# E3SM-Project/Omega

Hardware: AMD Instinct MI355X
Metric: tendency_cell_level_updates_per_sec (higher is better)
Workload: dtype f64

## Files before the change

### include/omega_amd.h

```cpp
#ifndef OMEGA_AMD_H
#define OMEGA_AMD_H

#include <stddef.h>
#include <stdint.h>

#ifdef __cplusplus
extern "C" {
#endif

typedef struct omg_decomp omg_decomp;
typedef struct omg_halo omg_halo;
typedef struct omg_mesh omg_mesh;
typedef struct omg_state omg_state;
typedef struct omg_tracers omg_tracers;
typedef struct omg_aux omg_aux;
typedef struct omg_tend omg_tend;
typedef struct omg_stepper omg_stepper;
typedef struct omg_vcoord omg_vcoord;
typedef struct omg_eos omg_eos;
typedef struct omg_vertmix omg_vertmix;
typedef struct omg_pgrad omg_pgrad;
typedef struct omg_vertadv omg_vertadv;

enum { OMG_ON_CELL = 0, OMG_ON_EDGE = 1, OMG_ON_VERTEX = 2 };
// ... 88 lines not shown
typedef struct omg_rccl omg_rccl;
int omg_rccl_get_unique_id(char *id );
int omg_rccl_create(const char *id, int nranks, int rank, omg_rccl **out);
int omg_rccl_destroy(omg_rccl *c);
int omg_rccl_abort(omg_rccl *c);
int omg_rccl_info(const omg_rccl *c, int *nranks, int *rank, int *version, int64_t *exchanges);
int omg_rccl_exchange(omg_rccl *c, int n, const int *peers, void *const *send_ptrs, const size_t *send_bytes,
                      void *const *recv_ptrs, const size_t *recv_bytes, void *stream);
int omg_halo_use_rccl(omg_halo *h, omg_rccl *c);
enum { OMG_PEER_HANDLE_BYTES = 160 };
typedef struct omg_peer omg_peer;
int omg_peer_create(int nranks, int rank, size_t mailbox_bytes, omg_peer **out);
int omg_peer_destroy(omg_peer *p);
int omg_peer_local_handle(const omg_peer *p, char *out );
int omg_peer_connect(omg_peer *p, const char *all_handles );
int omg_peer_info(const omg_peer *p, int64_t *exchanges, int *status);
int omg_peer_set_timeout(omg_peer *p, double seconds);
int omg_halo_use_peer(omg_halo *h, omg_peer *p);
int omg_halo_recv_rows(const omg_halo *h, size_t per_cell, size_t per_edge, size_t per_vertex, size_t *rows);
int omg_halo_exchange(omg_halo *h, double *dev_array, int nt, int rows_size, int k, int row_pitch, int elem,
                      void *stream);
int omg_halo_exchange_bytes(omg_halo *h, void *dev_array, int elem_bytes, int nt, int rows_size, int k, int row_pitch,
                            int elem, void *stream);
int omg_halo_exchange_i4(omg_halo *h, int32_t *dev_array, int nt, int rows_size, int k, int row_pitch, int elem,
                         void *stream);
int omg_halo_global_sum_dd(omg_halo *h, const double *local_hi_lo, int npairs, double *hi_lo, void *stream);
int omg_halo_exchange_state(omg_halo *h, omg_state *state, int state_time_level, omg_tracers *tracers,
                            int tracers_time_level, void *stream);
int omg_halo_check(const omg_halo *h);

int omg_set_option(const char *name, int value);
int omg_get_option(const char *name, int *value);
int omg_set_timing_level(int level);

int omg_mesh_create(const omg_decomp *d, int nvertlayers, int host_only, omg_mesh **out);
int omg_mesh_destroy(omg_mesh *m);
int omg_mesh_get_int(const omg_mesh *m, const char *name, int32_t *out);
int omg_mesh_get_array_i4(const omg_mesh *m, const char *name, int32_t *out, size_t n);
int omg_mesh_get_array_r8(const omg_mesh *m, const char *name, double *out, size_t n);
int omg_mesh_set_fvertex(omg_mesh *m, const double *host_values );

int omg_horz_divergence(const omg_mesh *m, const double *vec_edge_dev, double *div_cell_dev, int nvertlayers,
                        int row_pitch, int n, void *stream);
int omg_horz_gradient(const omg_mesh *m, const double *scalar_cell_dev, double *grad_edge_dev, int nvertlayers,
                      int row_pitch, int n, void *stream);
int omg_horz_curl(const omg_mesh *m, const double *vec_edge_dev, double *curl_vertex_dev, int nvertlayers,
                  int row_pitch, int n, void *stream);
int omg_horz_tangential_recon(const omg_mesh *m, const double *vec_edge_dev, double *recon_edge_dev, int nvertlayers,
                              int row_pitch, int n, void *stream);
int omg_horz_interp_cell_to_edge(const omg_mesh *m, const double *array_cell_dev, double *array_edge_dev,
                                 int isotropic, int n, void *stream);

typedef struct omg_tend_config {
   int32_t ThicknessFluxTendencyEnable, PVTendencyEnable, KETendencyEnable, SSHTendencyEnable,
       VelDiffTendencyEnable, VelHyperDiffTendencyEnable, WindForcingTendencyEnable, BottomDragTendencyEnable,
       TracerHorzAdvTendencyEnable, TracerDiffTendencyEnable, TracerHyperDiffTendencyEnable;
   int32_t FluxThicknessUpwind, FluxTracerUpwind, WindInterpIsotropic;
   double ViscDel2, ViscDel4, DivFactor, EddyDiff2, EddyDiff4, Density0, BottomDragCoeff;
} omg_tend_config;
void omg_tend_config_default(omg_tend_config *c);

int omg_state_create(const omg_mesh *m, omg_halo *halo, int nvertlayers, int ntimelevels, omg_state **out);
int omg_state_destroy(omg_state *s);
int omg_state_copy_to_device(omg_state *s, int time_level, const double *h_host, const double *u_host);
int omg_state_copy_to_host(const omg_state *s, int time_level, double *h_host, double *u_host);
int omg_state_device_ptr(const omg_state *s, int time_level, int which , double **dev);
// ... 172 lines not shown
```

### omega_amd/__init__.py

```python
from __future__ import annotations

import ctypes as C
import os
import subprocess

import numpy as np

_HERE = os.path.dirname(os.path.abspath(__file__))
LIB_PATH = os.environ.get("OMEGA_AMD_LIB", os.path.join(_HERE, "lib", "libomega_amd.so"))

ON_CELL, ON_EDGE, ON_VERTEX = 0, 1, 2

PD = C.POINTER(C.c_double)
PI = C.POINTER(C.c_int32)


class OmegaAmdError(RuntimeError):
    pass


def build(force: bool = False) -> str:
    cmd = ["make", "-C", os.path.join(_HERE, "csrc"), "-j8", "-s"]
    if force:
        cmd.append("-B")
# ... 20 lines not shown


class TendConfig(C.Structure):
    _fields_ = [(n, C.c_int32) for n in CONFIG_FLAGS] + [(n, C.c_double) for n in CONFIG_REALS]


TRANSPORT_FN = C.CFUNCTYPE(C.c_int, C.c_void_p, C.c_int, PI, C.POINTER(C.c_void_p), C.POINTER(C.c_size_t),
                           C.POINTER(C.c_void_p), C.POINTER(C.c_size_t), C.c_void_p)

CUSTOM_TEND_FN = C.CFUNCTYPE(C.c_int, C.c_void_p, C.c_void_p, C.c_void_p, C.c_void_p, C.c_int, C.c_int, C.c_int,
                             C.c_int, C.c_double, C.c_void_p)

_lib = None


def lib():
    global _lib
    if _lib is None:
        if not os.path.exists(LIB_PATH):
            raise OmegaAmdError(
                f"{LIB_PATH} not found: build it with `python -c 'import __graft_entry__ as g; g.build()'` "
                "(hipcc, gfx950). omega_amd has no CPU fallback.")
        L = C.CDLL(LIB_PATH)
        L.omg_last_error.restype = C.c_char_p
        _lib = L
        for item in filter(None, os.environ.get("OMEGA_AMD_OPTIONS", "").split(",")):
            name, _, val = item.partition("=")
            set_option(name.strip(), int(val))
    return _lib


def set_option(name: str, value: int):
    _chk(lib().omg_set_option(name.encode(), int(value)))


def get_option(name: str) -> int:
    v = C.c_int()
    _chk(lib().omg_get_option(name.encode(), C.byref(v)))
    return v.value


def _chk(rc):
    if rc != 0:
        raise OmegaAmdError(lib().omg_last_error().decode())


def _pd(a):
    if a is None:
        return PD()
    assert a.dtype == np.float64 and a.flags.c_contiguous, "need C-contiguous float64"
    return a.ctypes.data_as(PD)


def _pi(a):
    if a is None:
        return PI()
    assert a.dtype == np.int32 and a.flags.c_contiguous, "need C-contiguous int32"
    return a.ctypes.data_as(PI)


class _Handle:
    _destroy = None

    def _create(self, symbol: str, *args):
        h = C.c_void_p()
        _chk(getattr(lib(), symbol)(*args, C.byref(h)))
# ... 1171 lines not shown
```

### omega_amd/csrc/Device.cpp

```cpp
#include "Base.h"
#include "Pacer.h"
#include "Tuning.h"

#include <rocprofiler-sdk-roctx/roctx.h>

#include <atomic>
#include <cctype>
#include <cstdlib>

#include <cstring>
#include <sstream>

namespace OMEGA {

namespace {
struct OptionName {
   const char *Name;
   int TuningOptions::*Field;
};
const OptionName OptionTable[] = {
    {"MergeL1", &TuningOptions::MergeL1},
    {"Pair", &TuningOptions::Pair},
    {"TracerPatch", &TuningOptions::TracerPatch},
    {"SendBand", &TuningOptions::SendBand},
// ... 12 lines not shown
#ifdef OMEGA_TUNING_ENV
      for (const OptionName &O : OptionTable) {
         std::string Var = "OMEGA_";
         for (const char *C = O.Name; *C; ++C)
            Var += (char)std::toupper((unsigned char)*C);
         if (const char *V = std::getenv(Var.c_str()))
            X.*(O.Field) = std::atoi(V);
      }
#endif
      return X;
   }();
   return T;
}
namespace {
std::atomic<unsigned long long> TuningGen{0};
}
unsigned long long tuningGeneration() { return TuningGen.load(); }
bool setTuningOption(const std::string &Name, int Value) {
   for (const OptionName &O : OptionTable)
      if (Name == O.Name) {
         tuning().*(O.Field) = Value;
         ++TuningGen;
         return true;
      }
   return false;
}
bool getTuningOption(const std::string &Name, int &Value) {
   for (const OptionName &O : OptionTable)
      if (Name == O.Name) {
         Value = tuning().*(O.Field);
         return true;
      }
   return false;
}

namespace Pacer {
int &timingLevel() {
   static int Level = 3;
   return Level;
}
namespace {
constexpr int MaxLevels = 16;
thread_local int PushedAt[MaxLevels] = {};
int slot(int Level) { return Level < 0 ? 0 : (Level >= MaxLevels ? MaxLevels - 1 : Level); }
}
bool start(const char *Name, int Level) {
   if (Level <= timingLevel()) {
      roctxRangePushA(Name);
      if (Level > -1000000)
         ++PushedAt[slot(Level)];
   }
   return true;
}
bool stop(const char * , int Level) {
   if (Level <= -1000000) {
      roctxRangePop();
      return true;
   }
   if (PushedAt[slot(Level)] > 0) {
      --PushedAt[slot(Level)];
      roctxRangePop();
   }
   return true;
}
}

// ... 85 lines not shown
```

### omega_amd/csrc/Tuning.h

```cpp
#ifndef OMEGA_AMD_TUNING_H
#define OMEGA_AMD_TUNING_H

#include <string>

namespace OMEGA {

struct TuningOptions {
   int MergeL1 = 1;
   int Pair = 1;
   int TracerPatch = 1;
   int SendBand = 1;
   int BandOnComm = 1;
   int ShrinkSweeps = 1;
   int ForceGeneric = 0;
   int KeepMaxEdges = 0;
   int NarrowTables = 1;
   int Graphs = -1;
};

TuningOptions &tuning();
unsigned long long tuningGeneration();
bool setTuningOption(const std::string &Name, int Value);
bool getTuningOption(const std::string &Name, int &Value);

}
#endif
```

### omega_amd/csrc/capi.cpp

```cpp
#include "../../include/omega_amd.h"

#include "AuxiliaryState.h"
#include "Decomp.h"
#include "Halo.h"
#include "HorzMesh.h"
#include "HorzOperators.h"
#include "OceanState.h"
#include "Tendencies.h"
#include "CustomTendencyTerms.h"
#include "MeshIO.h"
#include "Partition.h"
#include "History.h"
#include "Pacer.h"
#include "PeerWire.h"
#include "Rccl.h"
#include "Tuning.h"
#include "TimeStepper.h"
#include "VertCoord.h"
#include "Eos.h"
#include "TriDiagSolvers.h"
#include "VertMix.h"
#include "PressureGrad.h"
#include "VertAdv.h"

// ... 544 lines not shown
   if (version)
      *version = c->C->Version;
   if (exchanges)
      *exchanges = c->C->NExchanges;
   OMG_CATCH
}
int omg_rccl_exchange(omg_rccl *c, int n, const int *peers, void *const *send_ptrs, const size_t *send_bytes,
                      void *const *recv_ptrs, const size_t *recv_bytes, void *stream) {
   OMG_TRY
   OMG_ARG(c && n >= 0 && (n == 0 || (peers && send_ptrs && send_bytes && recv_ptrs && recv_bytes)));
   if (c->C->exchange(n, peers, send_ptrs, send_bytes, recv_ptrs, recv_bytes, (hipStream_t)stream) != 0)
      OMEGA_ABORT(c->C->lastError());
   OMG_CATCH
}
int omg_halo_use_rccl(omg_halo *h, omg_rccl *c) {
   OMG_TRY
   OMG_ARG(h && c);
   h->H->useRccl(c->C.get());
   OMG_CATCH
}
int omg_set_option(const char *name, int value) {
   OMG_TRY
   OMG_ARG(name);
   if (!setTuningOption(name, value))
      OMEGA_ABORT(std::string("omg_set_option: no option named '") + name + "'");
   OMG_CATCH
}
int omg_get_option(const char *name, int *value) {
   OMG_TRY
   OMG_ARG(name && value);
   if (!getTuningOption(name, *value))
      OMEGA_ABORT(std::string("omg_get_option: no option named '") + name + "'");
   OMG_CATCH
}
int omg_set_timing_level(int level) {
   Pacer::timingLevel() = level;
   return 0;
}
int omg_peer_create(int nranks, int rank, size_t mailbox_bytes, omg_peer **out) {
   OMG_TRY
   OMG_ARG(out);
   newHandle(out, [&](omg_peer &R) { R.P.reset(new PeerWire(nranks, rank, mailbox_bytes)); });
   OMG_CATCH
}
int omg_peer_destroy(omg_peer *p) {
   delete p;
   return 0;
}
int omg_peer_local_handle(const omg_peer *p, char *out) {
   OMG_TRY
   OMG_ARG(p && out);
   p->P->localHandle(out);
   OMG_CATCH
}
int omg_peer_connect(omg_peer *p, const char *all_handles) {
   OMG_TRY
   OMG_ARG(p && all_handles);
   p->P->connect(all_handles);
   OMG_CATCH
}
int omg_peer_info(const omg_peer *p, int64_t *exchanges, int *status) {
   OMG_TRY
   OMG_ARG(p);
   if (exchanges)
      *exchanges = p->P->NExchanges;
   if (status)
// ... 1126 lines not shown
```

### omega_amd/csrc/kernels/KernelCommon.h

```cpp
#ifndef OMEGA_AMD_KERNELCOMMON_H
#define OMEGA_AMD_KERNELCOMMON_H

#include <cstdlib>
#include <type_traits>
#include <utility>
#include <hip/hip_runtime.h>

#include "../Base.h"
#include "../Tuning.h"

namespace OMEGA {

typedef double dv2 __attribute__((ext_vector_type(2)));

template <class T> struct VecW;
template <> struct VecW<double> {
   static constexpr int W = 1;
};
template <> struct VecW<dv2> {
   static constexpr int W = 2;
};

template <class T> __device__ __forceinline__ T ldk(const double *P, int Row, int K, int Kv) {
   return *reinterpret_cast<const T *>(P + (size_t)Row * K + (size_t)Kv * VecW<T>::W);
}
template <class T> __device__ __forceinline__ void stk(double *P, int Row, int K, int Kv, T V) {
   *reinterpret_cast<T *>(P + (size_t)Row * K + (size_t)Kv * VecW<T>::W) = V;
}

__device__ __forceinline__ double kmax(double A, double B) { return A < B ? B : A; }
__device__ __forceinline__ dv2 kmax(dv2 A, dv2 B) {
   dv2 R;
   R.x = kmax(A.x, B.x);
   R.y = kmax(A.y, B.y);
   return R;
}
__device__ __forceinline__ double upwind(double U, double A, double B) {
   return U > 0 ? A : (U < 0 ? B : kmax(A, B));
}
__device__ __forceinline__ dv2 upwind(dv2 U, dv2 A, dv2 B) {
   dv2 R;
   R.x = upwind(U.x, A.x, B.x);
   R.y = upwind(U.y, A.y, B.y);
   return R;
}
template <class T> __device__ __forceinline__ T splat(double V);
template <> __device__ __forceinline__ double splat<double>(double V) { return V; }
template <> __device__ __forceinline__ dv2 splat<dv2>(double V) {
   dv2 R;
   R.x = V;
   R.y = V;
   return R;
}

__device__ __forceinline__ double getc(double V, int) { return V; }
__device__ __forceinline__ double getc(dv2 V, int I) { return I == 0 ? V.x : V.y; }
__device__ __forceinline__ void setc(double &V, int, double X) { V = X; }
__device__ __forceinline__ void setc(dv2 &V, int I, double X) {
   if (I == 0)
      V.x = X;
   else
      V.y = X;
}

__device__ __forceinline__ int xcdRemap(int B, int N) {
   const int Q = N >> 3, R = N & 7;
   const int Xcd = B & 7, Idx = B >> 3;
   return (Xcd < R ? Xcd * (Q + 1) : R * (Q + 1) + (Xcd - R) * Q) + Idx;
}

struct LdsCarver {
   unsigned char *P;
   template <class U> __device__ __forceinline__ U *take(int N) {
      U *R = reinterpret_cast<U *>(P);
      P += (((size_t)N * sizeof(U) + 7) >> 3) << 3;
      return R;
   }
};
__host__ __device__ inline size_t ldsRound8(size_t B) { return ((B + 7) >> 3) << 3; }

struct Geom {
   dim3 Grid, Block;
   int KV;
   int Tile;
   int W;
   int NFull = 0, TailSplit = 1;
};
inline Geom makeGeom(int N, int K, int MaxW = 2, int Pitch = 0, int MaxTY = 0) {
   if (Pitch <= 0)
      Pitch = K;
   Geom G;
   G.W  = (K % 2 == 0 && MaxW >= 2) ? 2 : 1;
   G.KV = K / G.W;
   const int LineTX   = 128 / (8 * G.W);
   const bool Aligned = (Pitch * 8) % 128 == 0;
   int TX             = Aligned ? (G.KV < LineTX ? G.KV : LineTX) : (G.KV < 64 ? G.KV : 64);
   int TY = 256 / TX;
   while (MaxTY > 0 && TY > MaxTY && TY > 8)
      TY /= 2;
   while (TY > 8 && (N + TY - 1) / TY < 4096)
      TY /= 2;
   if (TY < 1)
      TY = 1;
   G.Block = dim3(TX, TY, 1);
   G.Tile  = TY;
   int NTiles = (N + G.Tile - 1) / G.Tile;
   int NChunks = (G.KV + TX - 1) / TX, Split = 1;
   while (Split < NChunks && (long)NTiles * Split < 1200)
      Split *= 2;
   if (Split > NChunks)
      Split = NChunks;
   G.Grid  = dim3(NTiles > 0 ? NTiles : 1, Split > 0 ? Split : 1, 1);
   G.NFull = NTiles;
   const int WavesPerWG     = (TX * TY + 63) / 64;
   const int Cap            = 256 * 8 / (WavesPerWG > 0 ? WavesPerWG : 1);
   if (Split == 1 && NChunks > 1 && NTiles >= Cap) {
      const int R = NTiles % Cap;
      if (R > 0) {
         G.NFull     = NTiles - R;
         G.TailSplit = NChunks;
         G.Grid      = dim3(G.NFull + R * NChunks, 1, 1);
      }
   }
   return G;
}

template <class B, class = void> struct BodyHoistTables {
   static constexpr bool V = false;
};
template <class B> struct BodyHoistTables<B, std::enable_if_t<B::HoistTables>> {
   static constexpr bool V = true;
};
template <class B> __device__ __forceinline__ void chunkFence() {
#ifndef OMEGA_NO_CHUNK_FENCE
   if constexpr (!BodyHoistTables<B>::V)
      __asm__ volatile("" ::: "memory");
#endif
}
template <class B, class = void> struct BodyOpaqueLe {
   static constexpr bool V = false;
};
template <class B> struct BodyOpaqueLe<B, std::enable_if_t<B::OpaqueLe>> {
   static constexpr bool V = true;
};
template <class B, class = void> struct BodyCooperative {
   static constexpr bool V = false;
};
template <class B> struct BodyCooperative<B, std::enable_if_t<B::Cooperative>> {
   static constexpr bool V = true;
};
template <class B, class = void> struct BodyMinWaves {
   static constexpr int V = 1;
};
template <class B> struct BodyMinWaves<B, decltype((void)B::MinWaves)> {
   static constexpr int V = B::MinWaves;
};
template <class B, class = void> struct BodyMaxW {
   static constexpr int V = 2;
// ... 20 lines not shown
   }
   const int First = TileId * Tile;
   int Cnt          = N - First;
   if (Cnt > Tile)
      Cnt = Tile;
   typename Body::Lds L = B.carve(Lds, Tile);
   const int Tid        = threadIdx.y * blockDim.x + threadIdx.x;
   const int NThr       = blockDim.x * blockDim.y;
   if (Cnt > 0)
      B.stage(L, First, Cnt, Tid, NThr);
   __syncthreads();
#ifdef OMEGA_STAGE_ONLY
   return;
#endif
   if constexpr (BodyCooperative<Body>::V) {
      B.template computeTile<T>(L, First, Cnt, C0, CS, KV);
   } else {
      for (int Le = threadIdx.y; Le < Cnt; Le += blockDim.y)
         for (int Kv = C0 * blockDim.x + threadIdx.x; Kv < KV; Kv += blockDim.x * CS) {
            chunkFence<Body>();
            if constexpr (BodyOpaqueLe<Body>::V) {
               int LeO = Le;
               __asm__ volatile("" : "+v"(LeO));
               B.template compute<T>(L, LeO, First + Le, Kv);
            } else
               B.template compute<T>(L, Le, First + Le, Kv);
         }
   }
}

template <class BA, class BB, class T>
__global__ void __launch_bounds__(OMEGA_LB, (BodyMinWaves<BA>::V < BodyMinWaves<BB>::V ? BodyMinWaves<BA>::V
                                                                                       : BodyMinWaves<BB>::V))
    tileKernel2(BA A, BB Bb, int NA, int NB, int KV, int Tile, int NTilesA, int NFullB, int TailSplit) {
   extern __shared__ __align__(16) unsigned char Lds[];
   const int Tid  = threadIdx.y * blockDim.x + threadIdx.x;
   const int NThr = blockDim.x * blockDim.y;
   if ((int)blockIdx.x < NTilesA) {
      const int Ta    = xcdRemap(blockIdx.x, NTilesA);
      const int First = Ta * Tile;
      const int Cnt   = NA - First < Tile ? NA - First : Tile;
      typename BA::Lds L = A.carve(Lds, Tile);
      if (Cnt > 0)
         A.stage(L, First, Cnt, Tid, NThr);
      __syncthreads();
#ifdef OMEGA_STAGE_ONLY
      return;
#endif
      for (int Le = threadIdx.y; Le < Cnt; Le += blockDim.y)
         for (int Kv = blockIdx.y * blockDim.x + threadIdx.x; Kv < KV; Kv += blockDim.x * gridDim.y)
         {
            chunkFence<BA>();
            A.template compute<T>(L, Le, First + Le, Kv);
         }
   } else {
      const int Bb_ = blockIdx.x - NTilesA;
      int TileId, C0 = blockIdx.y, CS = gridDim.y;
      if (Bb_ < NFullB) {
         TileId = xcdRemap(Bb_, NFullB);
      } else {
         TileId = NFullB + (Bb_ - NFullB) / TailSplit;
         C0     = (Bb_ - NFullB) % TailSplit;
         CS     = TailSplit;
      }
      const int First = TileId * Tile;
      const int Cnt   = NB - First < Tile ? NB - First : Tile;
      typename BB::Lds L = Bb.carve(Lds, Tile);
      if (Cnt > 0)
         Bb.stage(L, First, Cnt, Tid, NThr);
      __syncthreads();
#ifdef OMEGA_STAGE_ONLY
      return;
#endif
      for (int Le = threadIdx.y; Le < Cnt; Le += blockDim.y)
         for (int Kv = C0 * blockDim.x + threadIdx.x; Kv < KV; Kv += blockDim.x * CS)
         {
            chunkFence<BB>();
            Bb.template compute<T>(L, Le, First + Le, Kv);
         }
   }
}

template <class B, class = void> struct BodyHasNT {
   static constexpr bool V = false;
};
template <class B> struct BodyHasNT<B, decltype((void)std::declval<B &>().NT)> {
   static constexpr bool V = true;
};
template <class B> inline int bodyMaxTY(const B &Body) {
   if constexpr (BodyHasNT<B>::V)
      return Body.NT <= 8 ? 16 : 0;
   else
      return 0;
}
template <class B, class = void> struct BodyHasKLog {
   static constexpr bool V = false;
};
template <class B> struct BodyHasKLog<B, decltype((void)std::declval<B &>().KLog)> {
   static constexpr bool V = true;
};
template <class B, class = void> struct BodyHasNWv {
   static constexpr bool V = false;
};
template <class B> struct BodyHasNWv<B, decltype((void)std::declval<B &>().NWv)> {
   static constexpr bool V = true;
};
template <class B> inline void setWaves(B &Body, const Geom &G) {
   if constexpr (BodyHasNWv<B>::V)
      Body.NWv = (int)(G.Block.x * G.Block.y + 63) / 64;
}
template <class Body> void launchTile(const Body &B0, int N, int K, hipStream_t S, int Pitch = -1) {
   if (N <= 0)
      return;
   Body B = B0;
   B.K    = Pitch > 0 ? Pitch : levelPitch(K);
   if constexpr (BodyHasKLog<Body>::V)
      B.KLog = K;
   Geom G           = makeGeom(N, K, BodyMaxW<Body>::V, B.K, bodyMaxTY(B));
   setWaves(B, G);
   const size_t Lds = B.ldsBytes(G.Tile);
   if constexpr (BodyMaxW<Body>::V >= 2) {
      if (G.W == 2) {
         hipLaunchKernelGGL((tileKernel<Body, dv2>), G.Grid, G.Block, Lds, S, B, N, G.KV, G.Tile, G.NFull, G.TailSplit);
         HIP_CHECK(hipGetLastError());
         return;
      }
   }
   hipLaunchKernelGGL((tileKernel<Body, double>), G.Grid, G.Block, Lds, S, B, N, G.KV, G.Tile, G.NFull, G.TailSplit);
   HIP_CHECK(hipGetLastError());
}

template <class BA, class BB> void launchTile2(const BA &A0, int NA, const BB &B0, int NB, int K, hipStream_t S) {
   static_assert(BodyMaxW<BA>::V == BodyMaxW<BB>::V, "launchTile2: bodies must agree on the levels per thread");
   if (NA <= 0) {
      launchTile(B0, NB, K, S);
      return;
   }
   if (NB <= 0) {
      launchTile(A0, NA, K, S);
      return;
   }
   BA A  = A0;
   BB Bb = B0;
   A.K = Bb.K = levelPitch(K);
   if constexpr (BodyHasKLog<BA>::V)
      A.KLog = K;
   if constexpr (BodyHasKLog<BB>::V)
      Bb.KLog = K;
   const int TyA = bodyMaxTY(A), TyB = bodyMaxTY(Bb);
   Geom G        = makeGeom(NA + NB, K, BodyMaxW<BA>::V, A.K, TyA > TyB ? TyA : TyB);
   const int NTA = (NA + G.Tile - 1) / G.Tile, NTB = (NB + G.Tile - 1) / G.Tile;
   setWaves(A, G), setWaves(Bb, G);
   const size_t LA = A.ldsBytes(G.Tile), LB = Bb.ldsBytes(G.Tile), Lds = LA > LB ? LA : LB;
   int NFullB = NTB, TailSplit = 1;
   dim3 Grid(NTA + NTB, G.TailSplit > 1 ? 1 : G.Grid.y, 1);
   if (G.TailSplit > 1) {
      const int R = (NTA + NTB) - G.NFull;
      if (R > 0 && R <= NTB) {
         NFullB    = NTB - R;
         TailSplit = G.TailSplit;
         Grid      = dim3(NTA + NFullB + R * TailSplit, 1, 1);
      }
   }
   if constexpr (BodyMaxW<BA>::V >= 2) {
      if (G.W == 2) {
         hipLaunchKernelGGL((tileKernel2<BA, BB, dv2>), Grid, G.Block, Lds, S, A, Bb, NA, NB, G.KV, G.Tile, NTA, NFullB,
                            TailSplit);
         HIP_CHECK(hipGetLastError());
         return;
      }
   }
   hipLaunchKernelGGL((tileKernel2<BA, BB, double>), Grid, G.Block, Lds, S, A, Bb, NA, NB, G.KV, G.Tile, NTA, NFullB,
                      TailSplit);
   HIP_CHECK(hipGetLastError());
}

constexpr int MaxSweeps = 4;
struct SweepPlan {
   int N[MaxSweeps];
   int TileStart[MaxSweeps + 1];
};
template <int I, class T, class B, class... Rest>
__device__ __forceinline__ void runSweep(const SweepPlan &Pl, int KV, int Tile, unsigned char *Lds, const B &Body,
                                         const Rest &...More) {
   if ((int)blockIdx.x < Pl.TileStart[I + 1]) {
      const int NTiles = Pl.TileStart[I + 1] - Pl.TileStart[I];
      const int Tl     = xcdRemap(blockIdx.x - Pl.TileStart[I], NTiles);
      const int First  = Tl * Tile;
      const int Cnt    = Pl.N[I] - First < Tile ? Pl.N[I] - First : Tile;
      typename B::Lds L = Body.carve(Lds, Tile);
      const int Tid     = threadIdx.y * blockDim.x + threadIdx.x;
      if (Cnt > 0)
         Body.stage(L, First, Cnt, Tid, blockDim.x * blockDim.y);
      __syncthreads();
      if constexpr (BodyCooperative<B>::V) {
         Body.template computeTile<T>(L, First, Cnt, blockIdx.y, gridDim.y, KV);
      } else {
         for (int Le = threadIdx.y; Le < Cnt; Le += blockDim.y)
            for (int Kv = blockIdx.y * blockDim.x + threadIdx.x; Kv < KV; Kv += blockDim.x * gridDim.y) {
               chunkFence<B>();
               Body.template compute<T>(L, Le, First + Le, Kv);
            }
      }
      return;
   }
   if constexpr (sizeof...(Rest) > 0)
      runSweep<I + 1, T>(Pl, KV, Tile, Lds, More...);
}
template <class... Bs> struct MinWavesOf;
template <class B> struct MinWavesOf<B> {
   static constexpr int V = BodyMinWaves<B>::V;
};
template <class B, class... Bs> struct MinWavesOf<B, Bs...> {
   static constexpr int V = BodyMinWaves<B>::V < MinWavesOf<Bs...>::V ? BodyMinWaves<B>::V : MinWavesOf<Bs...>::V;
};
template <class T, class... Bs>
__global__ void __launch_bounds__(OMEGA_LB, MinWavesOf<Bs...>::V) tileKernelV(SweepPlan Pl, int KV, int Tile, Bs... Bodies) {
   extern __shared__ __align__(16) unsigned char Lds[];
   runSweep<0, T>(Pl, KV, Tile, Lds, Bodies...);
}

namespace detail {
template <class B> inline void prepBody(B &Body, int K) {
   Body.K = levelPitch(K);
   if constexpr (BodyHasKLog<B>::V)
      Body.KLog = K;
}
}
template <class B0, class B1> void launchTileV(int K, hipStream_t S, const B0 &A0, int N0, const B1 &A1, int N1) {
   static_assert(BodyMaxW<B0>::V == BodyMaxW<B1>::V, "launchTileV: bodies must agree on the levels per thread");
   static_assert(sizeof(B0) + sizeof(B1) + sizeof(SweepPlan) <= 3900, "launchTileV: kernel arguments exceed 4 KiB");
   B0 X0 = A0;
   B1 X1 = A1;
   detail::prepBody(X0, K), detail::prepBody(X1, K);
   const int Ns[2] = {N0 > 0 ? N0 : 0, N1 > 0 ? N1 : 0};
   const int Ty0 = bodyMaxTY(X0), Ty1 = bodyMaxTY(X1);
   Geom G = makeGeom(Ns[0] + Ns[1], K, BodyMaxW<B0>::V, X0.K, Ty0 > Ty1 ? Ty0 : Ty1);
   SweepPlan Pl{};
   Pl.TileStart[0] = 0;
   for (int I = 0; I < 2; ++I) {
      Pl.N[I]             = Ns[I];
      Pl.TileStart[I + 1] = Pl.TileStart[I] + (Ns[I] + G.Tile - 1) / G.Tile;
   }
   if (Pl.TileStart[2] == 0)
      return;
   setWaves(X0, G), setWaves(X1, G);
   const size_t L0 = X0.ldsBytes(G.Tile), L1 = X1.ldsBytes(G.Tile), Lds = L0 > L1 ? L0 : L1;
   const dim3 Grid(Pl.TileStart[2], G.TailSplit > 1 ? 1 : G.Grid.y, 1);
   if constexpr (BodyMaxW<B0>::V >= 2) {
      if (G.W == 2) {
         hipLaunchKernelGGL((tileKernelV<dv2, B0, B1>), Grid, G.Block, Lds, S, Pl, G.KV, G.Tile, X0, X1);
         HIP_CHECK(hipGetLastError());
         return;
      }
   }
   hipLaunchKernelGGL((tileKernelV<double, B0, B1>), Grid, G.Block, Lds, S, Pl, G.KV, G.Tile, X0, X1);
   HIP_CHECK(hipGetLastError());
}
template <class B0, class B1, class B2>
void launchTileV(int K, hipStream_t S, const B0 &A0, int N0, const B1 &A1, int N1, const B2 &A2, int N2) {
   static_assert(BodyMaxW<B0>::V == BodyMaxW<B1>::V && BodyMaxW<B0>::V == BodyMaxW<B2>::V,
                 "launchTileV: bodies must agree on the levels per thread");
   static_assert(sizeof(B0) + sizeof(B1) + sizeof(B2) + sizeof(SweepPlan) <= 3900, "launchTileV: kernel arguments exceed 4 KiB");
   B0 X0 = A0;
   B1 X1 = A1;
   B2 X2 = A2;
   detail::prepBody(X0, K), detail::prepBody(X1, K), detail::prepBody(X2, K);
   const int Ns[3] = {N0 > 0 ? N0 : 0, N1 > 0 ? N1 : 0, N2 > 0 ? N2 : 0};
   int Ty = bodyMaxTY(X0);
   Ty     = bodyMaxTY(X1) > Ty ? bodyMaxTY(X1) : Ty;
   Ty     = bodyMaxTY(X2) > Ty ? bodyMaxTY(X2) : Ty;
   Geom G = makeGeom(Ns[0] + Ns[1] + Ns[2], K, BodyMaxW<B0>::V, X0.K, Ty);
   SweepPlan Pl{};
   Pl.TileStart[0] = 0;
   for (int I = 0; I < 3; ++I) {
      Pl.N[I]             = Ns[I];
      Pl.TileStart[I + 1] = Pl.TileStart[I] + (Ns[I] + G.Tile - 1) / G.Tile;
   }
   if (Pl.TileStart[3] == 0)
      return;
   setWaves(X0, G), setWaves(X1, G), setWaves(X2, G);
   size_t Lds = X0.ldsBytes(G.Tile);
   Lds        = X1.ldsBytes(G.Tile) > Lds ? X1.ldsBytes(G.Tile) : Lds;
   Lds        = X2.ldsBytes(G.Tile) > Lds ? X2.ldsBytes(G.Tile) : Lds;
   const dim3 Grid(Pl.TileStart[3], G.TailSplit > 1 ? 1 : G.Grid.y, 1);
   if constexpr (BodyMaxW<B0>::V >= 2) {
      if (G.W == 2) {
         hipLaunchKernelGGL((tileKernelV<dv2, B0, B1, B2>), Grid, G.Block, Lds, S, Pl, G.KV, G.Tile, X0, X1, X2);
         HIP_CHECK(hipGetLastError());
         return;
      }
   }
   hipLaunchKernelGGL((tileKernelV<double, B0, B1, B2>), Grid, G.Block, Lds, S, Pl, G.KV, G.Tile, X0, X1, X2);
   HIP_CHECK(hipGetLastError());
}

}
#endif
```

Baseline: 7.858 billion.

## Size launch grids from measured occupancy and split tail tiles across all sweep kernels

Grid sizing now queries the HIP occupancy API, per kernel and LDS size, for the number of resident workgroups, instead of using a fixed nominal cap. The cached result drives both the chunk-split threshold, now a 3/5 fraction of capacity rather than a fixed 1200, and the tail-wave splitting. Tail splitting is extended to the multi-body sweep kernels (tileKernel2, tileKernelV), and bodies are ordered smallest first. The aim is fuller waves and less tail imbalance on the GPU, at the cost of a per-launch cache lookup plus more index arithmetic in the kernels.

```diff
diff --git a/include/omega_amd.h b/include/omega_amd.h
--- a/include/omega_amd.h
+++ b/include/omega_amd.h
@@ -144,6 +144,7 @@
 int omg_set_option(const char *name, int value);
 int omg_get_option(const char *name, int *value);
 int omg_set_timing_level(int level);
+int omg_set_launch_cap_for_tests(int cap);
 
 int omg_mesh_create(const omg_decomp *d, int nvertlayers, int host_only, omg_mesh **out);
 int omg_mesh_destroy(omg_mesh *m);
diff --git a/omega_amd/__init__.py b/omega_amd/__init__.py
--- a/omega_amd/__init__.py
+++ b/omega_amd/__init__.py
@@ -76,6 +76,10 @@
 
 def set_option(name: str, value: int):
     _chk(lib().omg_set_option(name.encode(), int(value)))
+
+
+def set_launch_cap_for_tests(cap: int):
+    _chk(lib().omg_set_launch_cap_for_tests(int(cap)))
 
 
 def get_option(name: str) -> int:
diff --git a/omega_amd/csrc/Device.cpp b/omega_amd/csrc/Device.cpp
--- a/omega_amd/csrc/Device.cpp
+++ b/omega_amd/csrc/Device.cpp
@@ -68,6 +68,11 @@
          return true;
       }
    return false;
+}
+
+int &launchCapOverride() {
+   static int Cap = 0;
+   return Cap;
 }
 
 namespace Pacer {
diff --git a/omega_amd/csrc/Tuning.h b/omega_amd/csrc/Tuning.h
--- a/omega_amd/csrc/Tuning.h
+++ b/omega_amd/csrc/Tuning.h
@@ -22,6 +22,7 @@
 unsigned long long tuningGeneration();
 bool setTuningOption(const std::string &Name, int Value);
 bool getTuningOption(const std::string &Name, int &Value);
+int &launchCapOverride();
 
 }
 #endif
diff --git a/omega_amd/csrc/capi.cpp b/omega_amd/csrc/capi.cpp
--- a/omega_amd/csrc/capi.cpp
+++ b/omega_amd/csrc/capi.cpp
@@ -600,6 +600,10 @@
    if (!getTuningOption(name, *value))
       OMEGA_ABORT(std::string("omg_get_option: no option named '") + name + "'");
    OMG_CATCH
+}
+int omg_set_launch_cap_for_tests(int cap) {
+   launchCapOverride() = cap > 0 ? cap : 0;
+   return 0;
 }
 int omg_set_timing_level(int level) {
    Pacer::timingLevel() = level;
diff --git a/omega_amd/csrc/kernels/KernelCommon.h b/omega_amd/csrc/kernels/KernelCommon.h
--- a/omega_amd/csrc/kernels/KernelCommon.h
+++ b/omega_amd/csrc/kernels/KernelCommon.h
@@ -4,10 +4,12 @@
 #include <cstdlib>
 #include <type_traits>
 #include <utility>
+#include <vector>
 #include <hip/hip_runtime.h>
 
 #include "../Base.h"
 #include "../Tuning.h"
+#include "LaunchGeometry.h"
 
 namespace OMEGA {
 
@@ -63,12 +65,6 @@
       V.y = X;
 }
 
-__device__ __forceinline__ int xcdRemap(int B, int N) {
-   const int Q = N >> 3, R = N & 7;
-   const int Xcd = B & 7, Idx = B >> 3;
-   return (Xcd < R ? Xcd * (Q + 1) : R * (Q + 1) + (Xcd - R) * Q) + Idx;
-}
-
 struct LdsCarver {
    unsigned char *P;
    template <class U> __device__ __forceinline__ U *take(int N) {
@@ -84,46 +80,69 @@
    int KV;
    int Tile;
    int W;
+   int NChunks;
    int NFull = 0, TailSplit = 1;
 };
-inline Geom makeGeom(int N, int K, int MaxW = 2, int Pitch = 0, int MaxTY = 0) {
-   if (Pitch <= 0)
-      Pitch = K;
+inline void setGrid(Geom &G, int NTiles, int Cap) {
+   const GridShape S = gridShape(NTiles, G.NChunks, Cap);
+   G.Grid            = dim3(S.GridX, S.Split, 1);
+   G.NFull           = NTiles > 0 ? S.NFull : 0;
+   G.TailSplit       = S.TailSplit;
+}
+inline Geom makeGeom(int N, int K, int MaxW = 2, int Pitch = 0, int MaxTY = 0, int Cap = 0) {
+   const TileShape T = tileShape(N, K, MaxW, Pitch, MaxTY);
    Geom G;
-   G.W  = (K % 2 == 0 && MaxW >= 2) ? 2 : 1;
-   G.KV = K / G.W;
-   const int LineTX   = 128 / (8 * G.W);
-   const bool Aligned = (Pitch * 8) % 128 == 0;
-   int TX             = Aligned ? (G.KV < LineTX ? G.KV : LineTX) : (G.KV < 64 ? G.KV : 64);
-   int TY = 256 / TX;
-   while (MaxTY > 0 && TY > MaxTY && TY > 8)
-      TY /= 2;
-   while (TY > 8 && (N + TY - 1) / TY < 4096)
-      TY /= 2;
-   if (TY < 1)
-      TY = 1;
-   G.Block = dim3(TX, TY, 1);
-   G.Tile  = TY;
-   int NTiles = (N + G.Tile - 1) / G.Tile;
-   int NChunks = (G.KV + TX - 1) / TX, Split = 1;
-   while (Split < NChunks && (long)NTiles * Split < 1200)
-      Split *= 2;
-   if (Split > NChunks)
-      Split = NChunks;
-   G.Grid  = dim3(NTiles > 0 ? NTiles : 1, Split > 0 ? Split : 1, 1);
-   G.NFull = NTiles;
-   const int WavesPerWG     = (TX * TY + 63) / 64;
-   const int Cap            = 256 * 8 / (WavesPerWG > 0 ? WavesPerWG : 1);
-   if (Split == 1 && NChunks > 1 && NTiles >= Cap) {
-      const int R = NTiles % Cap;
-      if (R > 0) {
-         G.NFull     = NTiles - R;
-         G.TailSplit = NChunks;
-         G.Grid      = dim3(G.NFull + R * NChunks, 1, 1);
-      }
-   }
+   G.W       = T.W;
+   G.KV      = T.KV;
+   G.Block   = dim3(T.TX, T.TY, 1);
+   G.Tile    = T.TY;
+   G.NChunks = T.NChunks;
+   setGrid(G, (N + G.Tile - 1) / G.Tile, Cap > 0 ? Cap : nominalCap(T.TX * T.TY));
    return G;
 }
+
+inline int residentWorkgroups(const void *F, int Threads, size_t Lds) {
+   if (launchCapOverride() > 0)
+      return launchCapOverride();
+   struct Entry {
+      const void *F;
+      int Threads, Device, Cap;
+      size_t Lds;
+   };
+   thread_local std::vector<Entry> Cache;
+   int Dev = 0;
+   if (hipGetDevice(&Dev) != hipSuccess)
+      Dev = -1;
+   for (const Entry &E : Cache)
+      if (E.F == F && E.Threads == Threads && E.Lds == Lds && E.Device == Dev)
+         return E.Cap;
+   int PerCU = 0, CUs = 0, Cap = nominalCap(Threads);
+   if (Dev >= 0 && hipOccupancyMaxActiveBlocksPerMultiprocessor(&PerCU, F, Threads, Lds) == hipSuccess &&
+       hipDeviceGetAttribute(&CUs, hipDeviceAttributeMultiprocessorCount, Dev) == hipSuccess && PerCU > 0 && CUs > 0)
+      Cap = PerCU * CUs;
+   else
+      (void)hipGetLastError();
+   Cache.push_back(Entry{F, Threads, Dev, Cap, Lds});
+   return Cap;
+}
+#ifdef OMEGA_GEOM_TRACE
+inline void geomTrace(const char *Who, int N, const Geom &G, dim3 Grid, int NFull, int TailSplit, int Cap, size_t Lds) {
+   struct Seen {
+      const char *Who;
+      int N;
+   };
+   thread_local std::vector<Seen> Done;
+   for (const Seen &S : Done)
+      if (S.Who == Who && S.N == N)
+         return;
+   Done.push_back(Seen{Who, N});
+   fprintf(stderr, "[geom] N=%d tile=%d block=%ux%u grid=%ux%u nfull=%d tailsplit=%d nchunks=%d cap=%d lds=%zu :: %s\n", N,
+           G.Tile, G.Block.x, G.Block.y, Grid.x, Grid.y, NFull, TailSplit, G.NChunks, Cap, Lds, Who);
+}
+#define OMEGA_GEOM_TRACE_CALL(...) geomTrace(__PRETTY_FUNCTION__, __VA_ARGS__)
+#else
+#define OMEGA_GEOM_TRACE_CALL(...) ((void)0)
+#endif
 
 template <class B, class = void> struct BodyHoistTables {
    static constexpr bool V = false;
@@ -210,13 +229,13 @@
 template <class BA, class BB, class T>
 __global__ void __launch_bounds__(OMEGA_LB, (BodyMinWaves<BA>::V < BodyMinWaves<BB>::V ? BodyMinWaves<BA>::V
                                                                                        : BodyMinWaves<BB>::V))
-    tileKernel2(BA A, BB Bb, int NA, int NB, int KV, int Tile, int NTilesA, int NFullB, int TailSplit) {
+    tileKernel2(BA A, BB Bb, int NA, int NB, int KV, int Tile, BodyBlocks RA, BodyBlocks RB, int TailSplit) {
    extern __shared__ __align__(16) unsigned char Lds[];
    const int Tid  = threadIdx.y * blockDim.x + threadIdx.x;
    const int NThr = blockDim.x * blockDim.y;
-   if ((int)blockIdx.x < NTilesA) {
-      const int Ta    = xcdRemap(blockIdx.x, NTilesA);
-      const int First = Ta * Tile;
+   int TileId, C0, CS;
+   if (bodySlot(RA, TailSplit, blockIdx.x, blockIdx.y, gridDim.y, TileId, C0, CS)) {
+      const int First = TileId * Tile;
       const int Cnt   = NA - First < Tile ? NA - First : Tile;
       typename BA::Lds L = A.carve(Lds, Tile);
       if (Cnt > 0)
@@ -226,21 +245,12 @@
       return;
 #endif
       for (int Le = threadIdx.y; Le < Cnt; Le += blockDim.y)
-         for (int Kv = blockIdx.y * blockDim.x + threadIdx.x; Kv < KV; Kv += blockDim.x * gridDim.y)
+         for (int Kv = C0 * blockDim.x + threadIdx.x; Kv < KV; Kv += blockDim.x * CS)
          {
             chunkFence<BA>();
             A.template compute<T>(L, Le, First + Le, Kv);
          }
-   } else {
-      const int Bb_ = blockIdx.x - NTilesA;
-      int TileId, C0 = blockIdx.y, CS = gridDim.y;
-      if (Bb_ < NFullB) {
-         TileId = xcdRemap(Bb_, NFullB);
-      } else {
-         TileId = NFullB + (Bb_ - NFullB) / TailSplit;
-         C0     = (Bb_ - NFullB) % TailSplit;
-         CS     = TailSplit;
-      }
+   } else if (bodySlot(RB, TailSplit, blockIdx.x, blockIdx.y, gridDim.y, TileId, C0, CS)) {
       const int First = TileId * Tile;
       const int Cnt   = NB - First < Tile ? NB - First : Tile;
       typename BB::Lds L = Bb.carve(Lds, Tile);
@@ -294,18 +304,23 @@
    B.K    = Pitch > 0 ? Pitch : levelPitch(K);
    if constexpr (BodyHasKLog<Body>::V)
       B.KLog = K;
-   Geom G           = makeGeom(N, K, BodyMaxW<Body>::V, B.K, bodyMaxTY(B));
+   Geom G = makeGeom(N, K, BodyMaxW<Body>::V, B.K, bodyMaxTY(B));
    setWaves(B, G);
    const size_t Lds = B.ldsBytes(G.Tile);
+   auto Go          = [&](auto Kern) {
+      const int Cap = residentWorkgroups(reinterpret_cast<const void *>(Kern), G.Block.x * G.Block.y, Lds);
+      setGrid(G, (N + G.Tile - 1) / G.Tile, Cap);
+      OMEGA_GEOM_TRACE_CALL(N, G, G.Grid, G.NFull, G.TailSplit, Cap, Lds);
+      hipLaunchKernelGGL(Kern, G.Grid, G.Block, Lds, S, B, N, G.KV, G.Tile, G.NFull, G.TailSplit);
+      HIP_CHECK(hipGetLastError());
+   };
    if constexpr (BodyMaxW<Body>::V >= 2) {
       if (G.W == 2) {
-         hipLaunchKernelGGL((tileKernel<Body, dv2>), G.Grid, G.Block, Lds, S, B, N, G.KV, G.Tile, G.NFull, G.TailSplit);
-         HIP_CHECK(hipGetLastError());
+         Go(&tileKernel<Body, dv2>);
          return;
       }
    }
-   hipLaunchKernelGGL((tileKernel<Body, double>), G.Grid, G.Block, Lds, S, B, N, G.KV, G.Tile, G.NFull, G.TailSplit);
-   HIP_CHECK(hipGetLastError());
+   Go(&tileKernel<Body, double>);
 }
 
 template <class BA, class BB> void launchTile2(const BA &A0, int NA, const BB &B0, int NB, int K, hipStream_t S) {
@@ -326,44 +341,38 @@
    if constexpr (BodyHasKLog<BB>::V)
       Bb.KLog = K;
    const int TyA = bodyMaxTY(A), TyB = bodyMaxTY(Bb);
-   Geom G        = makeGeom(NA + NB, K, BodyMaxW<BA>::V, A.K, TyA > TyB ? TyA : TyB);
-   const int NTA = (NA + G.Tile - 1) / G.Tile, NTB = (NB + G.Tile - 1) / G.Tile;
+   const Geom G  = makeGeom(NA + NB, K, BodyMaxW<BA>::V, A.K, TyA > TyB ? TyA : TyB);
    setWaves(A, G), setWaves(Bb, G);
    const size_t LA = A.ldsBytes(G.Tile), LB = Bb.ldsBytes(G.Tile), Lds = LA > LB ? LA : LB;
-   int NFullB = NTB, TailSplit = 1;
-   dim3 Grid(NTA + NTB, G.TailSplit > 1 ? 1 : G.Grid.y, 1);
-   if (G.TailSplit > 1) {
-      const int R = (NTA + NTB) - G.NFull;
-      if (R > 0 && R <= NTB) {
-         NFullB    = NTB - R;
-         TailSplit = G.TailSplit;
-         Grid      = dim3(NTA + NFullB + R * TailSplit, 1, 1);
-      }
-   }
+   auto Go = [&](auto Kern) {
+      const int Cap      = residentWorkgroups(reinterpret_cast<const void *>(Kern), G.Block.x * G.Block.y, Lds);
+      const int NTs[2]   = {(NA + G.Tile - 1) / G.Tile, (NB + G.Tile - 1) / G.Tile};
+      const int Order[2] = {0, 1};
+      const LaunchPlan P = planLaunch(NTs, Order, 2, G.NChunks, Cap);
+      const dim3 Grid(P.GridX, P.GridY, 1);
+      OMEGA_GEOM_TRACE_CALL(NA + NB, G, Grid, P.R[0].NFull + P.R[1].NFull, P.TailSplit, Cap, Lds);
+      hipLaunchKernelGGL(Kern, Grid, G.Block, Lds, S, A, Bb, NA, NB, G.KV, G.Tile, P.R[0], P.R[1], P.TailSplit);
+      HIP_CHECK(hipGetLastError());
+   };
    if constexpr (BodyMaxW<BA>::V >= 2) {
       if (G.W == 2) {
-         hipLaunchKernelGGL((tileKernel2<BA, BB, dv2>), Grid, G.Block, Lds, S, A, Bb, NA, NB, G.KV, G.Tile, NTA, NFullB,
-                            TailSplit);
-         HIP_CHECK(hipGetLastError());
+         Go(&tileKernel2<BA, BB, dv2>);
          return;
       }
    }
-   hipLaunchKernelGGL((tileKernel2<BA, BB, double>), Grid, G.Block, Lds, S, A, Bb, NA, NB, G.KV, G.Tile, NTA, NFullB,
-                      TailSplit);
-   HIP_CHECK(hipGetLastError());
-}
-
-constexpr int MaxSweeps = 4;
+   Go(&tileKernel2<BA, BB, double>);
+}
+
 struct SweepPlan {
    int N[MaxSweeps];
-   int TileStart[MaxSweeps + 1];
+   BodyBlocks R[MaxSweeps];
+   int TailSplit;
 };
 template <int I, class T, class B, class... Rest>
 __device__ __forceinline__ void runSweep(const SweepPlan &Pl, int KV, int Tile, unsigned char *Lds, const B &Body,
                                          const Rest &...More) {
-   if ((int)blockIdx.x < Pl.TileStart[I + 1]) {
-      const int NTiles = Pl.TileStart[I + 1] - Pl.TileStart[I];
-      const int Tl     = xcdRemap(blockIdx.x - Pl.TileStart[I], NTiles);
+   int Tl, C0, CS;
+   if (bodySlot(Pl.R[I], Pl.TailSplit, blockIdx.x, blockIdx.y, gridDim.y, Tl, C0, CS)) {
       const int First  = Tl * Tile;
       const int Cnt    = Pl.N[I] - First < Tile ? Pl.N[I] - First : Tile;
       typename B::Lds L = Body.carve(Lds, Tile);
@@ -372,10 +381,10 @@
          Body.stage(L, First, Cnt, Tid, blockDim.x * blockDim.y);
       __syncthreads();
       if constexpr (BodyCooperative<B>::V) {
-         Body.template computeTile<T>(L, First, Cnt, blockIdx.y, gridDim.y, KV);
+         Body.template computeTile<T>(L, First, Cnt, C0, CS, KV);
       } else {
          for (int Le = threadIdx.y; Le < Cnt; Le += blockDim.y)
-            for (int Kv = blockIdx.y * blockDim.x + threadIdx.x; Kv < KV; Kv += blockDim.x * gridDim.y) {
+            for (int Kv = C0 * blockDim.x + threadIdx.x; Kv < KV; Kv += blockDim.x * CS) {
                chunkFence<B>();
                Body.template compute<T>(L, Le, First + Le, Kv);
             }
@@ -403,6 +412,21 @@
    Body.K = levelPitch(K);
    if constexpr (BodyHasKLog<B>::V)
       Body.KLog = K;
+}
+inline bool planSweeps(const int *Ns, int NB, const Geom &G, int Cap, SweepPlan &Pl, dim3 &Grid) {
+   int NTs[MaxSweeps], Order[MaxSweeps];
+   for (int I = 0; I < NB; ++I)
+      NTs[I] = (Ns[I] + G.Tile - 1) / G.Tile;
+   listsFirst(Ns, NB, Order);
+   const LaunchPlan P = planLaunch(NTs, Order, NB, G.NChunks, Cap);
+   Pl                 = SweepPlan{};
+   for (int I = 0; I < NB; ++I) {
+      Pl.N[I] = Ns[I];
+      Pl.R[I] = P.R[I];
+   }
+   Pl.TailSplit = P.TailSplit;
+   Grid         = dim3(P.GridX, P.GridY, 1);
+   return P.GridX > 0;
 }
 }
 template <class B0, class B1> void launchTileV(int K, hipStream_t S, const B0 &A0, int N0, const B1 &A1, int N1) {
@@ -412,28 +436,29 @@
    B1 X1 = A1;
    detail::prepBody(X0, K), detail::prepBody(X1, K);
    const int Ns[2] = {N0 > 0 ? N0 : 0, N1 > 0 ? N1 : 0};
+   if (Ns[0] + Ns[1] == 0)
+      return;
    const int Ty0 = bodyMaxTY(X0), Ty1 = bodyMaxTY(X1);
-   Geom G = makeGeom(Ns[0] + Ns[1], K, BodyMaxW<B0>::V, X0.K, Ty0 > Ty1 ? Ty0 : Ty1);
-   SweepPlan Pl{};
-   Pl.TileStart[0] = 0;
-   for (int I = 0; I < 2; ++I) {
-      Pl.N[I]             = Ns[I];
-      Pl.TileStart[I + 1] = Pl.TileStart[I] + (Ns[I] + G.Tile - 1) / G.Tile;
-   }
-   if (Pl.TileStart[2] == 0)
-      return;
+   const Geom G  = makeGeom(Ns[0] + Ns[1], K, BodyMaxW<B0>::V, X0.K, Ty0 > Ty1 ? Ty0 : Ty1);
    setWaves(X0, G), setWaves(X1, G);
    const size_t L0 = X0.ldsBytes(G.Tile), L1 = X1.ldsBytes(G.Tile), Lds = L0 > L1 ? L0 : L1;
-   const dim3 Grid(Pl.TileStart[2], G.TailSplit > 1 ? 1 : G.Grid.y, 1);
+   auto Go = [&](auto Kern) {
+      const int Cap = residentWorkgroups(reinterpret_cast<const void *>(Kern), G.Block.x * G.Block.y, Lds);
+      SweepPlan Pl;
+      dim3 Grid;
+      if (!detail::planSweeps(Ns, 2, G, Cap, Pl, Grid))
+         return;
+      OMEGA_GEOM_TRACE_CALL(Ns[0] + Ns[1], G, Grid, Pl.R[0].NFull + Pl.R[1].NFull, Pl.TailSplit, Cap, Lds);
+      hipLaunchKernelGGL(Kern, Grid, G.Block, Lds, S, Pl, G.KV, G.Tile, X0, X1);
+      HIP_CHECK(hipGetLastError());
+   };
    if constexpr (BodyMaxW<B0>::V >= 2) {
       if (G.W == 2) {
-         hipLaunchKernelGGL((tileKernelV<dv2, B0, B1>), Grid, G.Block, Lds, S, Pl, G.KV, G.Tile, X0, X1);
-         HIP_CHECK(hipGetLastError());
+         Go(&tileKernelV<dv2, B0, B1>);
          return;
       }
    }
-   hipLaunchKernelGGL((tileKernelV<double, B0, B1>), Grid, G.Block, Lds, S, Pl, G.KV, G.Tile, X0, X1);
-   HIP_CHECK(hipGetLastError());
+   Go(&tileKernelV<double, B0, B1>);
 }
 template <class B0, class B1, class B2>
 void launchTileV(int K, hipStream_t S, const B0 &A0, int N0, const B1 &A1, int N1, const B2 &A2, int N2) {
@@ -445,33 +470,34 @@
    B2 X2 = A2;
    detail::prepBody(X0, K), detail::prepBody(X1, K), detail::prepBody(X2, K);
    const int Ns[3] = {N0 > 0 ? N0 : 0, N1 > 0 ? N1 : 0, N2 > 0 ? N2 : 0};
+   if (Ns[0] + Ns[1] + Ns[2] == 0)
+      return;
    int Ty = bodyMaxTY(X0);
    Ty     = bodyMaxTY(X1) > Ty ? bodyMaxTY(X1) : Ty;
    Ty     = bodyMaxTY(X2) > Ty ? bodyMaxTY(X2) : Ty;
-   Geom G = makeGeom(Ns[0] + Ns[1] + Ns[2], K, BodyMaxW<B0>::V, X0.K, Ty);
-   SweepPlan Pl{};
-   Pl.TileStart[0] = 0;
-   for (int I = 0; I < 3; ++I) {
-      Pl.N[I]             = Ns[I];
-      Pl.TileStart[I + 1] = Pl.TileStart[I] + (Ns[I] + G.Tile - 1) / G.Tile;
-   }
-   if (Pl.TileStart[3] == 0)
-      return;
+   const Geom G = makeGeom(Ns[0] + Ns[1] + Ns[2], K, BodyMaxW<B0>::V, X0.K, Ty);
    setWaves(X0, G), setWaves(X1, G), setWaves(X2, G);
    size_t Lds = X0.ldsBytes(G.Tile);
    Lds        = X1.ldsBytes(G.Tile) > Lds ? X1.ldsBytes(G.Tile) : Lds;
    Lds        = X2.ldsBytes(G.Tile) > Lds ? X2.ldsBytes(G.Tile) : Lds;
-   const dim3 Grid(Pl.TileStart[3], G.TailSplit > 1 ? 1 : G.Grid.y, 1);
+   auto Go    = [&](auto Kern) {
+      const int Cap = residentWorkgroups(reinterpret_cast<const void *>(Kern), G.Block.x * G.Block.y, Lds);
+      SweepPlan Pl;
+      dim3 Grid;
+      if (!detail::planSweeps(Ns, 3, G, Cap, Pl, Grid))
+         return;
+      OMEGA_GEOM_TRACE_CALL(Ns[0] + Ns[1] + Ns[2], G, Grid, Pl.R[0].NFull + Pl.R[1].NFull + Pl.R[2].NFull, Pl.TailSplit, Cap, Lds);
+      hipLaunchKernelGGL(Kern, Grid, G.Block, Lds, S, Pl, G.KV, G.Tile, X0, X1, X2);
+      HIP_CHECK(hipGetLastError());
+   };
    if constexpr (BodyMaxW<B0>::V >= 2) {
       if (G.W == 2) {
-         hipLaunchKernelGGL((tileKernelV<dv2, B0, B1, B2>), Grid, G.Block, Lds, S, Pl, G.KV, G.Tile, X0, X1, X2);
-         HIP_CHECK(hipGetLastError());
+         Go(&tileKernelV<dv2, B0, B1, B2>);
          return;
       }
    }
-   hipLaunchKernelGGL((tileKernelV<double, B0, B1, B2>), Grid, G.Block, Lds, S, Pl, G.KV, G.Tile, X0, X1, X2);
-   HIP_CHECK(hipGetLastError());
-}
-
-}
-#endif
+   Go(&tileKernelV<double, B0, B1, B2>);
+}
+
+}
+#endif
diff --git a/omega_amd/csrc/kernels/LaunchGeometry.h b/omega_amd/csrc/kernels/LaunchGeometry.h
--- /dev/null
+++ b/omega_amd/csrc/kernels/LaunchGeometry.h
@@ -0,0 +1,146 @@
+#ifndef OMEGA_AMD_LAUNCHGEOMETRY_H
+#define OMEGA_AMD_LAUNCHGEOMETRY_H
+
+#if defined(__HIPCC__)
+#define OMEGA_HD __host__ __device__ __forceinline__
+#else
+#define OMEGA_HD inline
+#endif
+
+namespace OMEGA {
+
+OMEGA_HD int xcdRemap(int B, int N) {
+   const int Q = N >> 3, R = N & 7;
+   const int Xcd = B & 7, Idx = B >> 3;
+   return (Xcd < R ? Xcd * (Q + 1) : R * (Q + 1) + (Xcd - R) * Q) + Idx;
+}
+
+struct TileShape {
+   int W;
+   int KV;
+   int TX, TY;
+   int NChunks;
+};
+#ifndef OMEGA_GEOM_HALVE_BELOW
+#define OMEGA_GEOM_HALVE_BELOW 4096
+#endif
+inline TileShape tileShape(int N, int K, int MaxW, int Pitch, int MaxTY) {
+   if (Pitch <= 0)
+      Pitch = K;
+   TileShape T;
+   T.W  = (K % 2 == 0 && MaxW >= 2) ? 2 : 1;
+   T.KV = K / T.W;
+   const int LineTX   = 128 / (8 * T.W);
+   const bool Aligned = (Pitch * 8) % 128 == 0;
+   T.TX               = Aligned ? (T.KV < LineTX ? T.KV : LineTX) : (T.KV < 64 ? T.KV : 64);
+   if (T.TX < 1)
+      T.TX = 1;
+   T.TY = 256 / T.TX;
+   while (MaxTY > 0 && T.TY > MaxTY && T.TY > 8)
+      T.TY /= 2;
+   while (T.TY > 8 && (N + T.TY - 1) / T.TY < OMEGA_GEOM_HALVE_BELOW)
+      T.TY /= 2;
+   if (T.TY < 1)
+      T.TY = 1;
+   T.NChunks = (T.KV + T.TX - 1) / T.TX;
+   return T;
+}
+inline int nominalCap(int ThreadsPerWG) {
+   const int Waves = (ThreadsPerWG + 63) / 64;
+   return 256 * 8 / (Waves > 0 ? Waves : 1);
+}
+
+struct GridShape {
+   int Split;
+   int NFull;
+   int TailSplit;
+   int GridX;
+};
+#ifndef OMEGA_GEOM_SPLIT_NUM
+#define OMEGA_GEOM_SPLIT_NUM 3
+#define OMEGA_GEOM_SPLIT_DEN 5
+#endif
+inline GridShape gridShape(int NTiles, int NChunks, int Cap) {
+   if (NTiles < 1)
+      NTiles = 1;
+   if (NChunks < 1)
+      NChunks = 1;
+   if (Cap < 1)
+      Cap = 1;
+   GridShape G{1, NTiles, 1, NTiles};
+   while (G.Split < NChunks && (long)NTiles * G.Split * OMEGA_GEOM_SPLIT_DEN < (long)Cap * OMEGA_GEOM_SPLIT_NUM)
+      G.Split *= 2;
+   if (G.Split > NChunks)
+      G.Split = NChunks;
+   if (G.Split == 1 && NChunks > 1 && NTiles >= Cap) {
+      const int R = NTiles % Cap;
+      if (R > 0) {
+         G.NFull     = NTiles - R;
+         G.TailSplit = NChunks;
+         G.GridX     = G.NFull + R * NChunks;
+      }
+   }
+   return G;
+}
+
+struct BodyBlocks {
+   int FullLo, NFull, TailLo, NTailBlocks;
+};
+OMEGA_HD bool bodySlot(const BodyBlocks &R, int TailSplit, int Bx, int By, int GridY, int &TileId, int &C0, int &CS) {
+   const unsigned F = (unsigned)(Bx - R.FullLo), T = (unsigned)(Bx - R.TailLo);
+   if (F < (unsigned)R.NFull) {
+      TileId = xcdRemap((int)F, R.NFull);
+      C0     = By;
+      CS     = GridY;
+      return true;
+   }
+   if (T < (unsigned)R.NTailBlocks) {
+      TileId = R.NFull + (int)T / TailSplit;
+      C0     = (int)T % TailSplit;
+      CS     = TailSplit;
+      return true;
+   }
+   return false;
+}
+
+constexpr int MaxSweeps = 4;
+struct LaunchPlan {
+   BodyBlocks R[MaxSweeps];
+   int TailSplit, GridX, GridY;
+};
+inline LaunchPlan planLaunch(const int *NTilesOf, const int *Order, int NBodies, int NChunks, int Cap) {
+   LaunchPlan P{};
+   int Total = 0;
+   for (int I = 0; I < NBodies; ++I)
+      Total += NTilesOf[I] > 0 ? NTilesOf[I] : 0;
+   const GridShape G = gridShape(Total, NChunks, Cap);
+   const int NFull   = Total > 0 ? G.NFull : 0;
+   P.TailSplit       = G.TailSplit;
+   P.GridX           = Total > 0 ? G.GridX : 0;
+   P.GridY           = G.Split;
+   int Seen = 0, FullLo = 0, TailLo = NFull;
+   for (int J = 0; J < NBodies; ++J) {
+      const int I  = Order[J];
+      const int NT = NTilesOf[I] > 0 ? NTilesOf[I] : 0;
+      int Full     = NFull - Seen;
+      Full         = Full < 0 ? 0 : (Full > NT ? NT : Full);
+      P.R[I]       = BodyBlocks{FullLo, Full, TailLo, (NT - Full) * G.TailSplit};
+      FullLo += Full;
+      TailLo += (NT - Full) * G.TailSplit;
+      Seen += NT;
+   }
+   return P;
+}
+inline void listsFirst(const int *N, int NBodies, int *Order) {
+   for (int I = 0; I < NBodies; ++I)
+      Order[I] = I;
+   for (int I = 1; I < NBodies; ++I)
+      for (int J = I; J > 0 && N[Order[J]] < N[Order[J - 1]]; --J) {
+         const int T  = Order[J];
+         Order[J]     = Order[J - 1];
+         Order[J - 1] = T;
+      }
+}
+
+}
+#endif
```

Result: no change. 7.864 billion (median of 3 runs) (+0.1%).
